# davdwan21/Silent-Speech

Hardware: AMD Instinct MI355X
Metric: clips/sec (30-frame, fwd+bwd) (higher is better)
Workload: dtype f32; 1 GPU; BASELINE config 2: landmark (K=40, D=84) + 64x64 uint8 ROI CNN + 2-layer BiGRU(192), T=30, C=5, train step = fwd + CE(ls .05) + bwd + grad all-reduce + clip(1.0) + Adam, dropout on; batch_per_gpu=256, global_batch=256, frames=30, parallelism=dp1, micro_batches_in_flight=1

## Files before the change

### include/ss_hotpath.h

```cpp
#ifndef SS_HOTPATH_H
#define SS_HOTPATH_H

#include <stdint.h>

#ifdef __cplusplus
extern "C" {
#endif

typedef void* ss_stream_t;

enum ss_status {
  SS_OK = 0,
  SS_ERR_ARG = -1,
  SS_ERR_LAUNCH = -2,
  SS_ERR_UNSUPPORTED = -3
};

int ss_abi_version(void);
const char* ss_status_string(int status);

int ss_feature_fuse(const float* lm, const uint8_t* reset, int B, int T, int K, int w, int h, int a_left,
                    int a_right, int a_up, int a_lo, int variant, float* X, int ldx, float* center,
                    double* fourth, ss_stream_t stream);

// ... 220 lines not shown
                const float* beta, const float* w1, const float* b1, const float* w4, const float* b4, const int64_t* y,
                int B, int T, int D, int MID, int C, float ln_eps, float drop_p, uint64_t seed, uint64_t offset,
                float label_smoothing, float denom, float* attn, float* xhat, float* rstd, float* ln, float* mid,
                float* mid_d, float* logits, float* d_logits, float* loss_sum, int32_t* correct, ss_stream_t stream);
int ss_tail_fwd_w(const float* h, const int32_t* lengths, const float* w_score, const float* b_score, const float* gamma,
                  const float* beta, const float* w1, const float* b1, const float* w4, const float* b4, const int64_t* y,
                  int B, int T, int D, int MID, int C, float ln_eps, float drop_p, uint64_t seed, uint64_t offset,
                  float label_smoothing, const float* cw, const float* den, float* attn, float* xhat, float* rstd, float* ln,
                  float* mid, float* mid_d, float* logits, float* d_logits, float* loss_sum, int32_t* correct,
                  ss_stream_t stream);
int ss_tail_bwd(const float* h, const int32_t* lengths, const float* w_score, const float* gamma, const float* w1,
                const float* w4, const float* attn, const float* xhat, const float* rstd, const float* mid,
                const float* d_logits, int B, int T, int D, int MID, int C, float drop_p, uint64_t seed,
                uint64_t offset, float* d_mid, float* d_h, float* g_gamma, float* g_beta, float* g_wscore,
                float* g_bscore, float* col_part, ss_stream_t stream);

int ss_ce_ls_fwd_bwd(const float* logits, const int64_t* y, int B, int C, float label_smoothing, float denom,
                     float* d_logits, float* loss_sum, int32_t* correct, ss_stream_t stream);

int ss_ce_ls_w_fwd_bwd(const float* logits, const int64_t* y, int B, int C, float label_smoothing, const float* w,
                       const float* den, float* d_logits, float* loss_sum, int32_t* correct, ss_stream_t stream);
int ss_class_weight_sum(const int64_t* y, long n, const float* w, int C, float* out, ss_stream_t stream);

int ss_eval_accum(const float* logits, const int64_t* y, int B, int C, float label_smoothing, int first_row,
                  float* loss_sum, int32_t* correct, int32_t* confusion, int32_t* first_seen, int32_t* y_true_out,
                  int32_t* y_pred_out, int32_t* err_flag, ss_stream_t stream);

int ss_eval_accum_w(const float* logits, const int64_t* y, int B, int C, float label_smoothing, int first_row, const float* w,
                    float* loss_sum, float* wsum, int32_t* correct, int32_t* confusion, int32_t* first_seen,
                    int32_t* y_true_out, int32_t* y_pred_out, int32_t* err_flag, ss_stream_t stream);
// ... 15 lines not shown
```

### silent_speech_amd/_lib.py

```python
from __future__ import annotations

import ctypes as C
import os

import torch

_HERE = os.path.dirname(os.path.abspath(__file__))
LIB_PATH = os.environ.get("SS_HOTPATH_LIB", os.path.join(_HERE, "libss_hotpath.so"))

_vp = C.c_void_p
_i = C.c_int
_f = C.c_float
_l = C.c_long
_u64 = C.c_uint64
_d = C.c_double

SIGNATURES = {
    "ss_abi_version": [],
    "ss_status_string": [_i],
    "ss_feature_fuse": [_vp, _vp, _i, _i, _i, _i, _i, _i, _i, _i, _i, _i, _vp, _i, _vp, _vp, _vp],
    "ss_feature_fuse_stream": [_vp, _vp, _vp, _i, _i, _i, _i, _i, _i, _i, _i, _i, _i, _d, _d, _vp, _vp, _vp, _i, _vp, _vp, _vp, _vp],
    "ss_roi_norm": [_vp, _i, _i, _i, _vp, _vp, _vp],
    "ss_im2col3x3": [_vp, _i, _i, _i, _i, _vp, _i, _vp],
    "ss_relu_pool2": [_vp, _i, _i, _i, _i, _vp, _vp, _vp],
# ... 62 lines not shown
    "ss_ring_push": [_vp, _vp, _i, _i, _i, _i, _vp, _i, _vp, _vp, _vp, _vp, _vp, _vp],
    "ss_ring_window_map": [_vp, _i, _i, _vp, _vp, _vp, _vp, _vp],
    "ss_mouth_openness": [_vp, _i, _i, _i, _i, _i, _i, _i, _vp, _vp],
    "ss_mouth_gate": [_vp, _i, _vp, _d, _d, _d, _vp, _vp, _vp],
    "ss_clip_gate": [_vp, _i, _vp, _vp, _d, _i, _i, _i, _i, _vp, _i, _i, _vp, _vp, _vp, _vp, _vp, _vp, _vp],
    "ss_gru_fwd": [_vp, _vp, _vp, _vp, _vp, _vp, _i, _i, _i, _vp, _vp, _vp, _vp],
    "ss_gru_fwd_drop": [_vp, _vp, _vp, _vp, _vp, _vp, _i, _i, _i, _vp, _vp, _vp, _f, _u64, _u64, _vp, _vp],
    "ss_gru_sync_bytes": [_i, _i, _i, _vp],
    "ss_gru_bwd": [_vp, _vp, _vp, _vp, _vp, _vp, _i, _i, _i, _vp, _f, _u64, _u64, _vp, _vp, _vp, _vp, _vp, _vp],
    "ss_gru_bias_grad": [_vp, _i, _i, _vp, _vp, _vp, _vp, _vp],
    "ss_attn_pool_fwd": [_vp, _vp, _vp, _vp, _i, _i, _i, _vp, _vp, _vp],
    "ss_attn_pool_bwd": [_vp, _vp, _vp, _vp, _vp, _i, _i, _i, _vp, _vp, _vp, _vp],
    "ss_tail_fwd": [_vp] * 11 + [_i] * 5 + [_f, _f, _u64, _u64, _f, _f] + [_vp] * 10 + [_vp],
    "ss_tail_fwd_w": [_vp] * 11 + [_i] * 5 + [_f, _f, _u64, _u64, _f, _vp, _vp] + [_vp] * 10 + [_vp],
    "ss_tail_bwd": [_vp] * 11 + [_i] * 5 + [_f, _u64, _u64] + [_vp] * 7 + [_vp],
    "ss_layernorm_fwd": [_vp, _vp, _vp, _i, _i, _f, _vp, _vp, _vp, _vp],
    "ss_layernorm_bwd": [_vp, _vp, _vp, _vp, _i, _i, _vp, _vp, _vp, _vp],
    "ss_dropout": [_vp, _vp, _l, _f, _u64, _u64, _vp, _vp],
    "ss_ce_ls_fwd_bwd": [_vp, _vp, _i, _i, _f, _f, _vp, _vp, _vp, _vp],
    "ss_eval_accum": [_vp, _vp, _i, _i, _f, _i, _vp, _vp, _vp, _vp, _vp, _vp, _vp, _vp],
    "ss_ce_ls_w_fwd_bwd": [_vp, _vp, _i, _i, _f, _vp, _vp, _vp, _vp, _vp, _vp],
    "ss_class_weight_sum": [_vp, _l, _vp, _i, _vp, _vp],
    "ss_eval_accum_w": [_vp, _vp, _i, _i, _f, _i, _vp, _vp, _vp, _vp, _vp, _vp, _vp, _vp, _vp, _vp],
    "ss_softmax_topk": [_vp, _i, _i, _i, _vp, _vp, _vp],
    "ss_sumsq_f32": [_vp, _l, _vp, _vp],
    "ss_adam_clip": [_vp, _vp, _vp, _vp, _l, _vp, _f, _f, _f, _f, _f, _f, _i, _vp],
    "ss_copy_rows_f32": [_vp, _i, _vp, _i, _i, _i, _vp],
}
_RESTYPES = {"ss_status_string": C.c_char_p}

# ... 110 lines not shown
```

### silent_speech_amd/csrc/tail.hip

```cpp
#include "ss_common.h"
#include "ce_row.h"

namespace {

constexpr int TNT = 1024;
constexpr int NWT = TNT / 64;


__device__ __forceinline__ float drop_scale(long idx, float p, uint64_t seed, uint64_t offset) {
  if (p <= 0.f) return 1.f;
  uint32_t rnd[4];
  const uint64_t ctr = offset + (uint64_t)(idx >> 2);
  philox4((uint32_t)ctr, (uint32_t)(ctr >> 32), 0u, 0u, (uint32_t)seed, (uint32_t)(seed >> 32), rnd);
  const uint32_t thr = (uint32_t)((double)p * 4294967296.0);
  return rnd[idx & 3] >= thr ? 1.0f / (1.0f - p) : 0.f;
}

__device__ __forceinline__ float block_sum(float v, float* red) {
  v = wave_sum(v);
  __syncthreads();
  if ((threadIdx.x & 63) == 0) red[threadIdx.x >> 6] = v;
  __syncthreads();
  float s = 0.f;
#pragma unroll
// ... 7 lines not shown
  const float *w_score, *b_score, *gamma, *beta, *w1, *b1, *w4, *b4;
  const int64_t* y;
  int B, T, D, MID, C;
  float eps, drop_p, ls, denom;
  uint64_t seed, offset;
  float *attn, *xhat, *rstd, *ln, *mid, *mid_d, *logits, *d_logits, *loss_sum;
  int* correct;
  static constexpr bool weighted = false;
};

struct TailFwdParamsW : TailFwdParams {
  const float *cw, *den;
  static constexpr bool weighted = true;
};

template <class Params>
__global__ __launch_bounds__(TNT) void tail_fwd_kernel(Params p) {
  extern __shared__ __attribute__((aligned(16))) float sm[];
  __shared__ float red[2 * NWT];
  const int T = p.T, D = p.D, MID = p.MID, C = p.C;
  float* sc = sm;
  float* pooled = sc + T;
  float* lnv = pooled + D;
  float* midv = lnv + D;
  float* lg = midv + MID;
  const int b = blockIdx.x, tid = threadIdx.x, lane = tid & 63, wv = tid >> 6;
  const int len = p.lengths[b];
  const float* hb = p.h + (long)b * T * D;

  constexpr int PF_PASS = 2, PF_IT = 6, PF_CH = 4;
  float wreg[PF_PASS][4][PF_IT];
#pragma unroll
  for (int ps = 0; ps < PF_PASS; ++ps)
#pragma unroll
// ... 3 lines not shown
        const int o = 4 * wv + u + 4 * NWT * ps, d = lane + 64 * it;
        wreg[ps][u][it] = (o < MID && d < D) ? p.w1[(long)o * D + d] : 0.f;
      }

  const float bsc = p.b_score[0];
  for (int t = wv; t < T; t += NWT) {
    float s = -1e9f;
    if (t < len) {
      s = 0.f;
      float hv[PF_IT], sw[PF_IT];
#pragma unroll
      for (int it = 0; it < PF_IT; ++it) {
        const int d = lane + 64 * it;
        hv[it] = d < D ? hb[(long)t * D + d] : 0.f;
        sw[it] = d < D ? p.w_score[d] : 0.f;
      }
#pragma unroll
      for (int it = 0; it < PF_IT; ++it) s += hv[it] * sw[it];
      for (int d0 = lane + 64 * PF_IT; d0 < D; d0 += 64 * PF_CH) {
        float h2[PF_CH], w2[PF_CH];
#pragma unroll
        for (int it = 0; it < PF_CH; ++it) {
          const int d = d0 + 64 * it;
          h2[it] = d < D ? hb[(long)t * D + d] : 0.f;
          w2[it] = d < D ? p.w_score[d] : 0.f;
        }
#pragma unroll
        for (int it = 0; it < PF_CH; ++it) s += h2[it] * w2[it];
      }
      s = wave_sum(s) + bsc;
    }
    if (lane == 0) sc[t] = s;
  }
  __syncthreads();
  float m = -3.4e38f;
  for (int t = tid; t < T; t += TNT) m = fmaxf(m, sc[t]);
  m = wave_max(m);
  if (lane == 0) red[wv] = m;
  __syncthreads();
  m = red[0];
// ... 4 lines not shown
    const float e = expf(sc[t] - m);
    sc[t] = e;
    sum += e;
  }
  sum = block_sum(sum, red + NWT);
  const float inv = 1.0f / sum;
  for (int t = tid; t < T; t += TNT) {
    const float wt = sc[t] * inv;
    sc[t] = wt;
    if (p.attn) p.attn[(long)b * T + t] = wt;
  }
  __syncthreads();
  float s1 = 0.f;
  for (int d = tid; d < D; d += TNT) {
    float acc = 0.f;
    for (int t = 0; t < len; ++t) acc += sc[t] * hb[(long)t * D + d];
    pooled[d] = acc;
    s1 += acc;
  }
  const float mean = block_sum(s1, red) / D;
  float s2 = 0.f;
  for (int d = tid; d < D; d += TNT) {
    const float c = pooled[d] - mean;
    s2 += c * c;
  }
  const float rs = rsqrtf(block_sum(s2, red + NWT) / D + p.eps);
  for (int d = tid; d < D; d += TNT) {
    const float xh = (pooled[d] - mean) * rs;
    const float v = xh * p.gamma[d] + p.beta[d];
    lnv[d] = v;
    if (p.xhat) p.xhat[(long)b * D + d] = xh;
    if (p.ln) p.ln[(long)b * D + d] = v;
  }
  if (p.rstd && tid == 0) p.rstd[b] = rs;
  __syncthreads();
  float xv[PF_IT];
#pragma unroll
  for (int it = 0; it < PF_IT; ++it) xv[it] = (lane + 64 * it < D) ? lnv[lane + 64 * it] : 0.f;
  int ps = 0;
  for (int o0 = 4 * wv; o0 < MID; o0 += 4 * NWT, ++ps) {
    float acc[4] = {0.f, 0.f, 0.f, 0.f};
    if (ps < PF_PASS) {
#pragma unroll
      for (int it = 0; it < PF_IT; ++it)
#pragma unroll
        for (int u = 0; u < 4; ++u) acc[u] += (ps == 0 ? wreg[0][u][it] : wreg[1][u][it]) * xv[it];
    }
    for (int d0 = lane + (ps < PF_PASS ? 64 * PF_IT : 0); d0 < D; d0 += 64 * PF_CH) {
      float w2[PF_CH][4];
// ... 5 lines not shown
          w2[it][u] = (d < D && o0 + u < MID) ? p.w1[(long)(o0 + u) * D + d] : 0.f;
        }
#pragma unroll
      for (int it = 0; it < PF_CH; ++it) {
        const int d = d0 + 64 * it;
        const float x = d < D ? lnv[d] : 0.f;
#pragma unroll
        for (int u = 0; u < 4; ++u) acc[u] += w2[it][u] * x;
      }
    }
#pragma unroll
    for (int u = 0; u < 4; ++u) acc[u] = wave_sum(acc[u]);
    if (lane < 4 && o0 + lane < MID) {
      const int o = o0 + lane;
      const float a = relu_f((lane == 0 ? acc[0] : lane == 1 ? acc[1] : lane == 2 ? acc[2] : acc[3]) + p.b1[o]);
      const float ad = a * drop_scale((long)b * MID + o, p.drop_p, p.seed, p.offset);
      midv[o] = ad;
      if (p.mid) p.mid[(long)b * MID + o] = a;
      if (p.mid_d) p.mid_d[(long)b * MID + o] = ad;
    }
  }
  __syncthreads();
  for (int c = wv; c < C; c += NWT) {
    float acc = 0.f;
    const float* wr = p.w4 + (long)c * MID;
    for (int o = lane; o < MID; o += 64) acc += wr[o] * midv[o];
    acc = wave_sum(acc);
    if (lane == 0) {
      const float v = acc + p.b4[c];
      lg[c] = v;
      p.logits[(long)b * C + c] = v;
    }
  }
  if (!p.y) return;
  __syncthreads();
  if (wv == 0) {
    float* d_row = p.d_logits + (long)b * C;
    float denom = p.denom;
    const float* cw = nullptr;
    bool valid = true;
    if constexpr (Params::weighted) {
      denom = p.den[0];
      cw = p.cw;
      valid = p.y[b] >= 0 && p.y[b] < (int64_t)C;
    }
    if (valid) {
      const int yy = (int)p.y[b];
      int am;
      const float loss = ce_row_wave<Params::weighted>(lg, yy, C, lane, p.ls, cw, denom, d_row, &am);
      if (lane == 0) {
        if (p.loss_sum) atomicAdd(p.loss_sum, loss / denom);
        if (p.correct && am == yy) atomicAdd(p.correct, 1);
      }
    } else {
      for (int c = lane; c < C; c += 64) d_row[c] = 0.f;
    }
  }
}

struct TailBwdParams {
  const float* h;
  const int* lengths;
  const float *w_score, *gamma, *w1, *w4;
  const float *attn, *xhat, *rstd, *mid, *d_logits;
  int B, T, D, MID, C;
  float drop_p;
  uint64_t seed, offset;
  float *d_mid, *d_h, *g_gamma, *g_beta, *g_wscore, *g_bscore;
  float* col_part;
};

__global__ __launch_bounds__(TNT) void tail_bwd_kernel(TailBwdParams p) {
  extern __shared__ __attribute__((aligned(16))) float sm[];
  __shared__ float red[2 * NWT];
  const int T = p.T, D = p.D, MID = p.MID, C = p.C;
  float* dmid = sm;
  float* dp = dmid + MID;
  float* ds = dp + D;
  float* wt = ds + T;
  float* dl = wt + T;
  const int b = blockIdx.x, tid = threadIdx.x, lane = tid & 63, wv = tid >> 6;
  const int len = p.lengths[b];
  const float* hb = p.h + (long)b * T * D;

  for (int c = tid; c < C; c += TNT) dl[c] = p.d_logits[(long)b * C + c];
  for (int t = tid; t < T; t += TNT) wt[t] = p.attn[(long)b * T + t];
  __syncthreads();
  for (int o = tid; o < MID; o += TNT) {
    float acc = 0.f;
#pragma unroll 16
    for (int c = 0; c < C; ++c) acc += dl[c] * p.w4[(long)c * MID + o];
    acc *= drop_scale((long)b * MID + o, p.drop_p, p.seed, p.offset);
    if (p.mid[(long)b * MID + o] <= 0.f) acc = 0.f;
    dmid[o] = acc;
    p.d_mid[(long)b * MID + o] = acc;
  }
  __syncthreads();
  float s1 = 0.f, s2 = 0.f;
  for (int d = tid; d < D; d += TNT) {
    float acc = 0.f;
#pragma unroll 16
    for (int o = 0; o < MID; ++o) acc += dmid[o] * p.w1[(long)o * D + d];
    const float xh = p.xhat[(long)b * D + d];
    if (p.col_part) {
      p.col_part[((long)b * 3 + 0) * D + d] = acc * xh;
      p.col_part[((long)b * 3 + 1) * D + d] = acc;
    } else {
      atomicAdd(&p.g_gamma[d], acc * xh);
      atomicAdd(&p.g_beta[d], acc);
    }
    const float dxh = acc * p.gamma[d];
    dp[d] = dxh;
    s1 += dxh;
    s2 += dxh * xh;
  }
  s1 = block_sum(s1, red) / D;
  s2 = block_sum(s2, red + NWT) / D;
  const float rs = p.rstd[b];
  for (int d = tid; d < D; d += TNT) dp[d] = rs * (dp[d] - s1 - p.xhat[(long)b * D + d] * s2);
  __syncthreads();
  for (int t = wv; t < T; t += NWT) {
    float c = 0.f;
    if (t < len) {
      for (int d = lane; d < D; d += 64) c += hb[(long)t * D + d] * dp[d];
      c = wave_sum(c);
    }
    if (lane == 0) ds[t] = c;
  }
  __syncthreads();
  float part = 0.f;
  for (int t = tid; t < len; t += TNT) part += wt[t] * ds[t];
  const float dot = block_sum(part, red);
  for (int t = tid; t < T; t += TNT) ds[t] = (t < len) ? wt[t] * (ds[t] - dot) : 0.f;
  __syncthreads();
  for (int d = tid; d < D; d += TNT) {
    const float dpd = dp[d], wd = p.w_score[d];
    float gw = 0.f;
#pragma unroll 8
    for (int t = 0; t < len; ++t) gw += ds[t] * hb[(long)t * D + d];
    for (int t = 0; t < T; ++t) p.d_h[((long)b * T + t) * D + d] = (t < len) ? wt[t] * dpd + ds[t] * wd : 0.f;
    if (p.col_part) p.col_part[((long)b * 3 + 2) * D + d] = gw;
    else atomicAdd(&p.g_wscore[d], gw);
  }
  if (tid == 0) {
    float gb = 0.f;
    for (int t = 0; t < len; ++t) gb += ds[t];
    atomicAdd(p.g_bscore, gb);
  }
}

}

static int tail_fwd_launch(const float* h, const int32_t* lengths, const float* w_score, const float* b_score,
                           const float* gamma, const float* beta, const float* w1, const float* b1, const float* w4,
                           const float* b4, const int64_t* y, int B, int T, int D, int MID, int C, float ln_eps,
                           float drop_p, uint64_t seed, uint64_t offset, float label_smoothing, float denom,
                           const float* cw, const float* den, float* attn, float* xhat, float* rstd, float* ln, float* mid,
                           float* mid_d, float* logits, float* d_logits, float* loss_sum, int32_t* correct,
                           ss_stream_t stream) {
  SS_REQUIRE(h && lengths && w_score && b_score && gamma && beta && w1 && b1 && w4 && b4 && logits, SS_ERR_ARG);
  SS_REQUIRE(B > 0 && T > 0 && D > 0 && MID > 0 && C > 0 && drop_p >= 0.f && drop_p < 1.f, SS_ERR_ARG);
  SS_REQUIRE(!y || (d_logits && denom > 0.f), SS_ERR_ARG);
  const size_t lds = (size_t)(T + 2 * D + MID + C) * sizeof(float);
// ... 44 lines not shown
                           float* g_wscore, float* g_bscore, float* col_part, ss_stream_t stream) {
  SS_REQUIRE(h && lengths && w_score && gamma && w1 && w4 && attn && xhat && rstd && mid && d_logits, SS_ERR_ARG);
  SS_REQUIRE(d_mid && d_h && g_gamma && g_beta && g_wscore && g_bscore, SS_ERR_ARG);
  SS_REQUIRE(B > 0 && T > 0 && D > 0 && MID > 0 && C > 0 && drop_p >= 0.f && drop_p < 1.f, SS_ERR_ARG);
  const size_t lds = (size_t)(MID + D + 2 * T + C) * sizeof(float);
  SS_REQUIRE(lds <= 60 * 1024, SS_ERR_UNSUPPORTED);
  TailBwdParams p;
  p.h = h; p.lengths = lengths; p.w_score = w_score; p.gamma = gamma; p.w1 = w1; p.w4 = w4;
  p.attn = attn; p.xhat = xhat; p.rstd = rstd; p.mid = mid; p.d_logits = d_logits;
  p.B = B; p.T = T; p.D = D; p.MID = MID; p.C = C; p.drop_p = drop_p; p.seed = seed; p.offset = offset;
  p.d_mid = d_mid; p.d_h = d_h; p.g_gamma = g_gamma; p.g_beta = g_beta; p.g_wscore = g_wscore; p.g_bscore = g_bscore;
  p.col_part = col_part;
  hipLaunchKernelGGL(tail_bwd_kernel, dim3(B), dim3(TNT), lds, static_cast<hipStream_t>(stream), p);
  return ss_launch_status();
}
```

### silent_speech_amd/engine.py

```python
from __future__ import annotations

import os

from dataclasses import dataclass
from typing import Dict, Optional

import torch

from . import _lib as L

INT_MAX = 2**31 - 1
_HH_TARGET = 512
USE_SIDE_STREAM = True


@dataclass
class Config:
    x_dim: int
    num_classes: int
    use_roi: bool
    roi_emb: int = 32
    hidden: int = 192
    gru_layers: int = 2
    roi_standardize: bool = True
# ... 117 lines not shown
class Workspace:

    bf16 = False

    def __init__(self, cfg: Config, B: int, T: int, roi_hw, device, train: bool, slot=0):
        self.cfg, self.B, self.T, self.roi_hw, self.train = cfg, B, T, roi_hw, train
        self.stash_gen, self.stash_live = 0, False
        N, H = B * T, cfg.hidden
        f32 = dict(device=device, dtype=torch.float32)
        u8 = dict(device=device, dtype=torch.uint8)
        self.lengths = torch.empty(B, device=device, dtype=torch.int32)
        nb = L.gru_sync_bytes(B, T, H)
        self.gru_sync = torch.zeros(nb // 4, device=device, dtype=torch.int32) if nb else None
        self.side = side_stream(device, slot) if train else None
        self.ev_fork = torch.cuda.Event() if train else None
        self.ev_join = torch.cuda.Event() if train else None
        self.ev_cnn_fwd = torch.cuda.Event() if train else None
        self.stagger = False
        self.Z = torch.empty(N, cfg.in_dim, **f32) if cfg.use_roi and roi_hw is not None else None
        self.cnn_generic = None
        if cfg.use_roi and roi_hw is not None:
            from . import cnn_generic

            if not cnn_generic.fused_supported(*roi_hw):
                self.cnn_generic = cnn_generic.GenericCnn(N, roi_hw[0], roi_hw[1], device, train)
        self.gi = [torch.empty(2, N, 3 * H, **f32) for _ in range(cfg.gru_layers)]
        self.out = [torch.empty(N, 2 * H, **f32) for _ in range(cfg.gru_layers)]
        self.attn = torch.empty(B, T, **f32)
        self.pooled = torch.empty(B, 2 * H, **f32)
        self.ln = torch.empty(B, 2 * H, **f32)
# ... 27 lines not shown
                n_a1, n_a2, n_i1, n_i2, n_m3, n_feat = self.cnn_sizes
                self.st_a1 = torch.empty(N, n_a1, **f32)
                self.st_i1 = torch.empty(N, n_i1, **u8)
                self.st_a2 = torch.empty(N, n_a2, **f32)
                self.st_i2 = torch.empty(N, n_i2, **u8)
                self.st_m3 = torch.empty(N, n_m3, **u8)
                self.st_feat = torch.empty(N, n_feat, **f32)
        self.frames = (torch.empty(1 + N, device=device, dtype=torch.int32)
                       if cfg.use_roi and roi_hw is not None and self.cnn_generic is None and SKIP_PADDED_FRAMES else None)
        self.frames_seen = (torch.full((1,), -1, dtype=torch.int32).pin_memory()
                            if self.frames is not None and train else None)
        self.walk_listed = self.frames is not None


def forward(P: Dict[str, torch.Tensor], cfg: Config, ws: Workspace, X: torch.Tensor, R: Optional[torch.Tensor], *,
            train: bool, stash: bool = False, seed: int = 0, ce=None, x_in_place: bool = False, z_ready: bool = False) -> torch.Tensor:
    if ws.bf16:
        from . import engine_bf16

        return engine_bf16.forward(P, cfg, ws, X, R, train=train, stash=stash, seed=seed, ce=ce, x_in_place=x_in_place)
    B, T, H, N = ws.B, ws.T, cfg.hidden, ws.B * ws.T
    s = L.stream()
    if stash and not ws.train:
        raise RuntimeError("stash=True needs a training workspace")
    if z_ready:
        if stash or train or not cfg.use_roi or X.shape[2] != cfg.in_dim:
            raise RuntimeError("z_ready: inference on rows of width in_dim = x_dim + roi_emb of a use_roi model")
        layer_in, ld_in = X.data_ptr(), cfg.in_dim
    elif cfg.use_roi:
        Hh, Ww = ws.roi_hw
        ws_Z = ws.Z
# ... 30 lines not shown
        fused_drop = drop and ws.gru_sync is not None
        L.call("ss_gru_fwd_drop", ws.gi[l].data_ptr(), P[f"gru.weight_hh_l{l}"].data_ptr(),
               P[f"gru.weight_hh_l{l}_reverse"].data_ptr(), P[f"gru.bias_hh_l{l}"].data_ptr(),
               P[f"gru.bias_hh_l{l}_reverse"].data_ptr(), ws.lengths.data_ptr(), B, T, H, ws.out[l].data_ptr(),
               ws.save[l].data_ptr() if stash else None, ws.out_drop[l].data_ptr() if fused_drop else None,
               cfg.gru_dropout if fused_drop else 0.0, seed, (l + 1) << 40, L.ptr(ws.gru_sync), s, tag="ss_gru_fwd")
        layer_in, ld_in = ws.out[l].data_ptr(), 2 * H
        if drop:
            if not fused_drop:
                L.call("ss_dropout", ws.out[l].data_ptr(), ws.out_drop[l].data_ptr(), N * 2 * H, cfg.gru_dropout, seed,
                       (l + 1) << 40, None, s)
            layer_in = ws.out_drop[l].data_ptr()
    top = ws.out[cfg.gru_layers - 1]
    p_drop = cfg.head_dropout if train else 0.0
    y_ptr, ls, denom, loss_ptr, correct_ptr, cw_ptr, den_ptr = (tuple(ce) + (None, None))[:7] if ce is not None else (None, 0.0, 1.0, None, None, None, None)
    tail_fwd, ce_norm = ("ss_tail_fwd_w", (cw_ptr, den_ptr)) if cw_ptr else ("ss_tail_fwd", (denom,))
    L.call(tail_fwd, top.data_ptr(), ws.lengths.data_ptr(), P["pool.score.weight"].data_ptr(),
           P["pool.score.bias"].data_ptr(), P["head.0.weight"].data_ptr(), P["head.0.bias"].data_ptr(),
           P["head.1.weight"].data_ptr(), P["head.1.bias"].data_ptr(), P["head.4.weight"].data_ptr(),
           P["head.4.bias"].data_ptr(), y_ptr, B, T, 2 * H, cfg.head_mid, cfg.num_classes, cfg.ln_eps, p_drop, seed,
           7 << 40, ls, *ce_norm, ws.attn.data_ptr() if stash else None, ws.xhat.data_ptr() if stash else None,
           ws.rstd.data_ptr() if stash else None, ws.ln.data_ptr() if stash else None,
           ws.mid.data_ptr() if stash else None, ws.mid_drop.data_ptr() if stash else None, ws.logits.data_ptr(),
           ws.d_logits.data_ptr() if ce is not None else None, loss_ptr, correct_ptr, s)
    return ws.logits


def backward(P: Dict[str, torch.Tensor], G: Dict[str, torch.Tensor], cfg: Config, ws: Workspace, X: torch.Tensor,
             R: Optional[torch.Tensor], d_logits: torch.Tensor, *, train: bool, seed: int = 0,
             d_X: Optional[torch.Tensor] = None) -> None:
    if ws.bf16:
        from . import engine_bf16

        return engine_bf16.backward(P, G, cfg, ws, X, R, d_logits, train=train, seed=seed, d_X=d_X)
    B, T, H, N = ws.B, ws.T, cfg.hidden, ws.B * ws.T
    s = L.stream()
    C, MID = cfg.num_classes, cfg.head_mid
    p_drop = cfg.head_dropout if train else 0.0
    top = ws.out[cfg.gru_layers - 1]
    L.call("ss_tail_bwd", top.data_ptr(), ws.lengths.data_ptr(), P["pool.score.weight"].data_ptr(),
           P["head.0.weight"].data_ptr(), P["head.1.weight"].data_ptr(), P["head.4.weight"].data_ptr(),
           ws.attn.data_ptr(), ws.xhat.data_ptr(), ws.rstd.data_ptr(), ws.mid.data_ptr(), d_logits.data_ptr(), B, T,
           2 * H, MID, C, p_drop, seed, 7 << 40, ws.d_mid.data_ptr(), ws.d_out.data_ptr(),
           G["head.0.weight"].data_ptr(), G["head.0.bias"].data_ptr(), G["pool.score.weight"].data_ptr(),
           G["pool.score.bias"].data_ptr(), ws.tail_part.data_ptr(), s)
    side = ws.side if USE_SIDE_STREAM else torch.cuda.current_stream()
    ws.ev_fork.record()

    def head_side_work():
        with torch.cuda.stream(side):
            side.wait_event(ws.ev_fork)
            zero_buffers(ws.d_lower[1:] + ([ws.dZ] if cfg.use_roi else []))
            ws.ev_zero.record()
            if ws.frames_seen is not None:
                ws.frames_seen.copy_(ws.frames[:1], non_blocking=True)
            for k_, name_ in enumerate(("head.0.weight", "head.0.bias", "pool.score.weight")):
                L.call("ss_colsum_f32", _addr(ws.tail_part, k_ * 2 * H), B, 2 * H, 3 * 2 * H, G[name_].data_ptr(), L.stream())
            gemm(0, 0, C, MID, B, d_logits.data_ptr(), C, ws.mid_drop.data_ptr(), MID, G["head.4.weight"].data_ptr(), MID,
                 accumulate=True, atomic=True, a_colsum=G["head.4.bias"].data_ptr())
            gemm(0, 0, MID, 2 * H, B, ws.d_mid.data_ptr(), MID, ws.ln.data_ptr(), 2 * H, G["head.1.weight"].data_ptr(),
                 2 * H, accumulate=True, atomic=True, a_colsum=G["head.1.bias"].data_ptr())

    use_drop = train and cfg.gru_dropout > 0.0
    zero_waited = False
    for l in range(cfg.gru_layers - 1, -1, -1):
        K = cfg.in_dim if l == 0 else 2 * H
# ... 70 lines not shown
```

### silent_speech_amd/train.py

```python
from __future__ import annotations

from typing import Optional

import numpy as np
import torch

from . import _lib as L
from . import engine as E
from .model import BiGRUClassifier


def shard_range(n_items: int, rank: int, world: int):
    per = (n_items + world - 1) // world
    lo = min(n_items, rank * per)
    return lo, min(n_items, lo + per)


def allreduce_flat_grads(flat: torch.Tensor, group=None, always: bool = False) -> None:
    import torch.distributed as dist

    if dist.is_available() and dist.is_initialized() and (always or dist.get_world_size(group) > 1):
        dist.all_reduce(flat, op=dist.ReduceOp.SUM, group=group)


# ... 6 lines not shown
        w64 = np.asarray(class_weights, dtype=np.float64)
    except (TypeError, ValueError) as e:
        raise ValueError(f"class_weights must be a sequence of {num_classes} numbers") from e
    if w64.shape != (num_classes,):
        raise ValueError(f"class_weights must hold one weight per class: shape ({num_classes},), not {w64.shape}")
    with np.errstate(over="ignore"):
        w = w64.astype(np.float32)
    if not (np.isfinite(w).all() and (w > 0).all()):
        raise ValueError("class_weights must be finite and strictly positive")
    return np.ascontiguousarray(w)


class Trainer:

    CNN_RESERVED_CUS = 32

    def __init__(self, model: BiGRUClassifier, lr: float = 3e-4, max_norm: float = 1.0,
                 label_smoothing: float = 0.05, betas=(0.9, 0.999), eps: float = 1e-8, world_size: int = 1,
                 process_group=None, dropout: bool = True, micro_batches: int = 1, always_allreduce: bool = False,
                 class_weights=None):
        cw = None if class_weights is None else check_class_weights(class_weights, model.cfg.num_classes)
        if model.flat_params is None or not model.flat_params.is_cuda:
            raise RuntimeError("Trainer needs the model on a HIP device")
        L.load()
        self.model, self.lr, self.max_norm, self.ls = model, lr, max_norm, label_smoothing
        self.betas, self.eps = betas, eps
        self.world, self.group = world_size, process_group
        self.always_allreduce = always_allreduce
        self.allreduce_events = None
        self.dropout = dropout
# ... 105 lines not shown
        n_el = model.flat_grads.numel()
        L.call("ss_sumsq_f32", model.flat_grads.data_ptr(), n_el, self.scal.data_ptr() + 4, s)
        L.call("ss_adam_clip", model.flat_params.data_ptr(), model.flat_grads.data_ptr(), self.m.data_ptr(),
               self.v.data_ptr(), n_el, self.scal.data_ptr() + 4, 1.0, self.max_norm, self.lr, self.betas[0],
               self.betas[1], self.eps, self.step_count, s)
        return self.scal[0], self.correct[0]

    def _fwd_bwd(self, X, lengths, R, y, denom, train, seed, slot, phase, prologue_done=False):
        model, cfg = self.model, self.model.cfg
        ws = model._workspace(X, R, train=True, slot=slot)
        P = model._param_dict()
        if phase in ("fwd", "both"):
            if not prologue_done:
                ws.lengths.copy_(lengths.to(torch.int32), non_blocking=True)
            E.forward(P, cfg, ws, X, R, train=train, stash=True, seed=seed, x_in_place=prologue_done,
                      ce=(y.data_ptr(), self.ls, denom, self.scal.data_ptr(), self.correct.data_ptr()) + self._ce_w)
        if phase in ("bwd", "both"):
            E.backward(P, self.G, cfg, ws, X, R, ws.d_logits, train=train, seed=seed)

    def grad_norm(self) -> torch.Tensor:
        return self.scal[1].sqrt()
```

Measured before the change: 133,900 clips/s.

## Fuse tail forward, loss and tail backward into one kernel

Adds a combined tail training kernel that runs the attention pooling, LayerNorm, MLP head, label-smoothed CE and the tail backward in one block per sample. Intermediates such as xhat, rstd, mid, the dropout keep mask and d_logits stay in LDS instead of going through global memory. When LDS allows, the sample's hidden rows are also cached in LDS so the three later passes over h skip global reads. This removes a kernel launch and the stash writes and reads, and avoids recomputing the Philox dropout mask. In exchange the kernel asks for up to 128KB of dynamic LDS per block, which may lower occupancy. Backward then waits on a new event instead of launching the tail backward itself.

```diff
diff --git a/include/ss_hotpath.h b/include/ss_hotpath.h
--- a/include/ss_hotpath.h
+++ b/include/ss_hotpath.h
@@ -258,6 +258,19 @@
                 const float* d_logits, int B, int T, int D, int MID, int C, float drop_p, uint64_t seed,
                 uint64_t offset, float* d_mid, float* d_h, float* g_gamma, float* g_beta, float* g_wscore,
                 float* g_bscore, float* col_part, ss_stream_t stream);
+int ss_tail_train(const float* h, const int32_t* lengths, const float* w_score, const float* b_score, const float* gamma,
+                  const float* beta, const float* w1, const float* b1, const float* w4, const float* b4, const int64_t* y,
+                  int B, int T, int D, int MID, int C, float ln_eps, float drop_p, uint64_t seed, uint64_t offset,
+                  float label_smoothing, float denom, float* attn, float* xhat, float* rstd, float* ln, float* mid,
+                  float* mid_d, float* logits, float* d_logits, float* loss_sum, int32_t* correct, float* d_mid, float* d_h,
+                  float* g_gamma, float* g_beta, float* g_wscore, float* g_bscore, float* col_part, ss_stream_t stream);
+int ss_tail_train_w(const float* h, const int32_t* lengths, const float* w_score, const float* b_score, const float* gamma,
+                    const float* beta, const float* w1, const float* b1, const float* w4, const float* b4, const int64_t* y,
+                    int B, int T, int D, int MID, int C, float ln_eps, float drop_p, uint64_t seed, uint64_t offset,
+                    float label_smoothing, const float* cw, const float* den, float* attn, float* xhat, float* rstd,
+                    float* ln, float* mid, float* mid_d, float* logits, float* d_logits, float* loss_sum, int32_t* correct,
+                    float* d_mid, float* d_h, float* g_gamma, float* g_beta, float* g_wscore, float* g_bscore,
+                    float* col_part, ss_stream_t stream);
 
 int ss_ce_ls_fwd_bwd(const float* logits, const int64_t* y, int B, int C, float label_smoothing, float denom,
                      float* d_logits, float* loss_sum, int32_t* correct, ss_stream_t stream);
diff --git a/silent_speech_amd/_lib.py b/silent_speech_amd/_lib.py
--- a/silent_speech_amd/_lib.py
+++ b/silent_speech_amd/_lib.py
@@ -100,6 +100,8 @@
     "ss_tail_fwd": [_vp] * 11 + [_i] * 5 + [_f, _f, _u64, _u64, _f, _f] + [_vp] * 10 + [_vp],
     "ss_tail_fwd_w": [_vp] * 11 + [_i] * 5 + [_f, _f, _u64, _u64, _f, _vp, _vp] + [_vp] * 10 + [_vp],
     "ss_tail_bwd": [_vp] * 11 + [_i] * 5 + [_f, _u64, _u64] + [_vp] * 7 + [_vp],
+    "ss_tail_train": [_vp] * 11 + [_i] * 5 + [_f, _f, _u64, _u64, _f, _f] + [_vp] * 10 + [_vp] * 7 + [_vp],
+    "ss_tail_train_w": [_vp] * 11 + [_i] * 5 + [_f, _f, _u64, _u64, _f, _vp, _vp] + [_vp] * 10 + [_vp] * 7 + [_vp],
     "ss_layernorm_fwd": [_vp, _vp, _vp, _i, _i, _f, _vp, _vp, _vp, _vp],
     "ss_layernorm_bwd": [_vp, _vp, _vp, _vp, _i, _i, _vp, _vp, _vp, _vp],
     "ss_dropout": [_vp, _vp, _l, _f, _u64, _u64, _vp, _vp],
diff --git a/silent_speech_amd/csrc/tail.hip b/silent_speech_amd/csrc/tail.hip
--- a/silent_speech_amd/csrc/tail.hip
+++ b/silent_speech_amd/csrc/tail.hip
@@ -45,10 +45,13 @@
   static constexpr bool weighted = true;
 };
 
-template <class Params>
-__global__ __launch_bounds__(TNT) void tail_fwd_kernel(Params p) {
-  extern __shared__ __attribute__((aligned(16))) float sm[];
-  __shared__ float red[2 * NWT];
+struct TailHand {
+  float *xhat, *rstd, *mid, *scale, *dl, *hs;
+};
+
+
+template <class Params, int MODE>
+__device__ __forceinline__ void tail_fwd_body(const Params& p, float* sm, float* red, const TailHand& hd) {
   const int T = p.T, D = p.D, MID = p.MID, C = p.C;
   float* sc = sm;
   float* pooled = sc + T;
@@ -82,6 +85,7 @@
         const int d = lane + 64 * it;
         hv[it] = d < D ? hb[(long)t * D + d] : 0.f;
         sw[it] = d < D ? p.w_score[d] : 0.f;
+        if (MODE == 2 && d < D) hd.hs[t * D + d] = hv[it];
       }
 #pragma unroll
       for (int it = 0; it < PF_IT; ++it) s += hv[it] * sw[it];
@@ -92,6 +96,7 @@
           const int d = d0 + 64 * it;
           h2[it] = d < D ? hb[(long)t * D + d] : 0.f;
           w2[it] = d < D ? p.w_score[d] : 0.f;
+          if (MODE == 2 && d < D) hd.hs[t * D + d] = h2[it];
         }
 #pragma unroll
         for (int it = 0; it < PF_CH; ++it) s += h2[it] * w2[it];
@@ -126,7 +131,11 @@
   float s1 = 0.f;
   for (int d = tid; d < D; d += TNT) {
     float acc = 0.f;
-    for (int t = 0; t < len; ++t) acc += sc[t] * hb[(long)t * D + d];
+    if (MODE == 2) {
+      for (int t = 0; t < len; ++t) acc += sc[t] * hd.hs[t * D + d];
+    } else {
+      for (int t = 0; t < len; ++t) acc += sc[t] * hb[(long)t * D + d];
+    }
     pooled[d] = acc;
     s1 += acc;
   }
@@ -141,10 +150,12 @@
     const float xh = (pooled[d] - mean) * rs;
     const float v = xh * p.gamma[d] + p.beta[d];
     lnv[d] = v;
+    if (MODE > 0) hd.xhat[d] = xh;
     if (p.xhat) p.xhat[(long)b * D + d] = xh;
     if (p.ln) p.ln[(long)b * D + d] = v;
   }
   if (p.rstd && tid == 0) p.rstd[b] = rs;
+  if (MODE > 0 && tid == 0) hd.rstd[0] = rs;
   __syncthreads();
   float xv[PF_IT];
 #pragma unroll
@@ -180,8 +191,13 @@
     if (lane < 4 && o0 + lane < MID) {
       const int o = o0 + lane;
       const float a = relu_f((lane == 0 ? acc[0] : lane == 1 ? acc[1] : lane == 2 ? acc[2] : acc[3]) + p.b1[o]);
-      const float ad = a * drop_scale((long)b * MID + o, p.drop_p, p.seed, p.offset);
+      const float keep = drop_scale((long)b * MID + o, p.drop_p, p.seed, p.offset);
+      const float ad = a * keep;
       midv[o] = ad;
+      if (MODE > 0) {
+        hd.mid[o] = a;
+        hd.scale[o] = keep;
+      }
       if (p.mid) p.mid[(long)b * MID + o] = a;
       if (p.mid_d) p.mid_d[(long)b * MID + o] = ad;
     }
@@ -201,7 +217,8 @@
   if (!p.y) return;
   __syncthreads();
   if (wv == 0) {
-    float* d_row = p.d_logits + (long)b * C;
+    float* d_out_row = p.d_logits + (long)b * C;
+    float* d_row = MODE > 0 ? hd.dl : d_out_row;
     float denom = p.denom;
     const float* cw = nullptr;
     bool valid = true;
@@ -221,7 +238,16 @@
     } else {
       for (int c = lane; c < C; c += 64) d_row[c] = 0.f;
     }
-  }
+    if (MODE > 0)
+      for (int c = lane; c < C; c += 64) d_out_row[c] = d_row[c];
+  }
+}
+
+template <class Params>
+__global__ __launch_bounds__(TNT) void tail_fwd_kernel(Params p) {
+  extern __shared__ __attribute__((aligned(16))) float sm[];
+  __shared__ float red[2 * NWT];
+  tail_fwd_body<Params, 0>(p, sm, red, TailHand{});
 }
 
 struct TailBwdParams {
@@ -236,28 +262,29 @@
   float* col_part;
 };
 
-__global__ __launch_bounds__(TNT) void tail_bwd_kernel(TailBwdParams p) {
-  extern __shared__ __attribute__((aligned(16))) float sm[];
-  __shared__ float red[2 * NWT];
+template <int MODE>
+__device__ __forceinline__ void tail_bwd_body(const TailBwdParams& p, float* sm, float* wt, float* dl, float* red,
+                                              const TailHand& hd) {
   const int T = p.T, D = p.D, MID = p.MID, C = p.C;
   float* dmid = sm;
   float* dp = dmid + MID;
   float* ds = dp + D;
-  float* wt = ds + T;
-  float* dl = wt + T;
   const int b = blockIdx.x, tid = threadIdx.x, lane = tid & 63, wv = tid >> 6;
   const int len = p.lengths[b];
   const float* hb = p.h + (long)b * T * D;
-
-  for (int c = tid; c < C; c += TNT) dl[c] = p.d_logits[(long)b * C + c];
-  for (int t = tid; t < T; t += TNT) wt[t] = p.attn[(long)b * T + t];
+  const float* xrow = MODE > 0 ? hd.xhat : p.xhat + (long)b * D;
+
+  if (MODE == 0) {
+    for (int c = tid; c < C; c += TNT) dl[c] = p.d_logits[(long)b * C + c];
+    for (int t = tid; t < T; t += TNT) wt[t] = p.attn[(long)b * T + t];
+  }
   __syncthreads();
   for (int o = tid; o < MID; o += TNT) {
     float acc = 0.f;
 #pragma unroll 16
     for (int c = 0; c < C; ++c) acc += dl[c] * p.w4[(long)c * MID + o];
-    acc *= drop_scale((long)b * MID + o, p.drop_p, p.seed, p.offset);
-    if (p.mid[(long)b * MID + o] <= 0.f) acc = 0.f;
+    acc *= MODE > 0 ? hd.scale[o] : drop_scale((long)b * MID + o, p.drop_p, p.seed, p.offset);
+    if ((MODE > 0 ? hd.mid[o] : p.mid[(long)b * MID + o]) <= 0.f) acc = 0.f;
     dmid[o] = acc;
     p.d_mid[(long)b * MID + o] = acc;
   }
@@ -267,7 +294,7 @@
     float acc = 0.f;
 #pragma unroll 16
     for (int o = 0; o < MID; ++o) acc += dmid[o] * p.w1[(long)o * D + d];
-    const float xh = p.xhat[(long)b * D + d];
+    const float xh = xrow[d];
     if (p.col_part) {
       p.col_part[((long)b * 3 + 0) * D + d] = acc * xh;
       p.col_part[((long)b * 3 + 1) * D + d] = acc;
@@ -282,13 +309,17 @@
   }
   s1 = block_sum(s1, red) / D;
   s2 = block_sum(s2, red + NWT) / D;
-  const float rs = p.rstd[b];
-  for (int d = tid; d < D; d += TNT) dp[d] = rs * (dp[d] - s1 - p.xhat[(long)b * D + d] * s2);
+  const float rs = MODE > 0 ? hd.rstd[0] : p.rstd[b];
+  for (int d = tid; d < D; d += TNT) dp[d] = rs * (dp[d] - s1 - xrow[d] * s2);
   __syncthreads();
   for (int t = wv; t < T; t += NWT) {
     float c = 0.f;
     if (t < len) {
-      for (int d = lane; d < D; d += 64) c += hb[(long)t * D + d] * dp[d];
+      if (MODE == 2) {
+        for (int d = lane; d < D; d += 64) c += hd.hs[t * D + d] * dp[d];
+      } else {
+        for (int d = lane; d < D; d += 64) c += hb[(long)t * D + d] * dp[d];
+      }
       c = wave_sum(c);
     }
     if (lane == 0) ds[t] = c;
@@ -302,8 +333,13 @@
   for (int d = tid; d < D; d += TNT) {
     const float dpd = dp[d], wd = p.w_score[d];
     float gw = 0.f;
+    if (MODE == 2) {
 #pragma unroll 8
-    for (int t = 0; t < len; ++t) gw += ds[t] * hb[(long)t * D + d];
+      for (int t = 0; t < len; ++t) gw += ds[t] * hd.hs[t * D + d];
+    } else {
+#pragma unroll 8
+      for (int t = 0; t < len; ++t) gw += ds[t] * hb[(long)t * D + d];
+    }
     for (int t = 0; t < T; ++t) p.d_h[((long)b * T + t) * D + d] = (t < len) ? wt[t] * dpd + ds[t] * wd : 0.f;
     if (p.col_part) p.col_part[((long)b * 3 + 2) * D + d] = gw;
     else atomicAdd(&p.g_wscore[d], gw);
@@ -313,6 +349,42 @@
     for (int t = 0; t < len; ++t) gb += ds[t];
     atomicAdd(p.g_bscore, gb);
   }
+}
+
+__global__ __launch_bounds__(TNT) void tail_bwd_kernel(TailBwdParams p) {
+  extern __shared__ __attribute__((aligned(16))) float sm[];
+  __shared__ float red[2 * NWT];
+  float* wt = sm + p.MID + p.D + p.T;
+  tail_bwd_body<0>(p, sm, wt, wt + p.T, red, TailHand{});
+}
+
+struct TailTrainParams {
+  TailFwdParamsW f;
+  TailBwdParams g;
+};
+
+constexpr size_t tail_train_lds_floats(int T, int D, int MID, int C) {
+  return (size_t)(T + 2 * D + MID + C) + D + 2 * MID + C + 4 + (MID + D + T);
+}
+
+template <bool WEIGHTED, bool KEEP>
+__global__ __launch_bounds__(TNT) void tail_train_kernel(TailTrainParams p) {
+  extern __shared__ __attribute__((aligned(16))) float sm[];
+  __shared__ float red[2 * NWT];
+  const int T = p.f.T, D = p.f.D, MID = p.f.MID, C = p.f.C;
+  constexpr int MODE = KEEP ? 2 : 1;
+  float* fwd = sm;
+  TailHand hd;
+  hd.xhat = fwd + T + 2 * D + MID + C;
+  hd.mid = hd.xhat + D;
+  hd.scale = hd.mid + MID;
+  hd.dl = hd.scale + MID;
+  hd.rstd = hd.dl + C;
+  float* bwd = hd.rstd + 4;
+  hd.hs = bwd + MID + D + T;
+  if constexpr (WEIGHTED) tail_fwd_body<TailFwdParamsW, MODE>(p.f, fwd, red, hd);
+  else tail_fwd_body<TailFwdParams, MODE>(static_cast<const TailFwdParams&>(p.f), fwd, red, hd);
+  tail_bwd_body<MODE>(p.g, bwd, fwd , hd.dl, red, hd);
 }
 
 }
@@ -387,3 +459,72 @@
   hipLaunchKernelGGL(tail_bwd_kernel, dim3(B), dim3(TNT), lds, static_cast<hipStream_t>(stream), p);
   return ss_launch_status();
 }
+
+constexpr int TAIL_TRAIN_LDS = 128 * 1024;
+
+template <bool WEIGHTED, bool KEEP>
+static int tail_train_go(const TailTrainParams& p, size_t lds, hipStream_t stream) {
+  const int st = ss_dynamic_lds(reinterpret_cast<const void*>(&tail_train_kernel<WEIGHTED, KEEP>), TAIL_TRAIN_LDS);
+  if (st != SS_OK) return st;
+  hipLaunchKernelGGL((tail_train_kernel<WEIGHTED, KEEP>), dim3(p.f.B), dim3(TNT), lds, stream, p);
+  return ss_launch_status();
+}
+
+static int tail_train_launch(const float* h, const int32_t* lengths, const float* w_score, const float* b_score,
+                             const float* gamma, const float* beta, const float* w1, const float* b1, const float* w4,
+                             const float* b4, const int64_t* y, int B, int T, int D, int MID, int C, float ln_eps,
+                             float drop_p, uint64_t seed, uint64_t offset, float label_smoothing, float denom,
+                             const float* cw, const float* den, float* attn, float* xhat, float* rstd, float* ln, float* mid,
+                             float* mid_d, float* logits, float* d_logits, float* loss_sum, int32_t* correct, float* d_mid,
+                             float* d_h, float* g_gamma, float* g_beta, float* g_wscore, float* g_bscore, float* col_part,
+                             ss_stream_t stream) {
+  SS_REQUIRE(h && lengths && w_score && b_score && gamma && beta && w1 && b1 && w4 && b4 && y && logits && d_logits, SS_ERR_ARG);
+  SS_REQUIRE(d_mid && d_h && g_gamma && g_beta && g_wscore && g_bscore, SS_ERR_ARG);
+  SS_REQUIRE(B > 0 && T > 0 && D > 0 && MID > 0 && C > 0 && drop_p >= 0.f && drop_p < 1.f && denom > 0.f, SS_ERR_ARG);
+  const size_t base = tail_train_lds_floats(T, D, MID, C) * sizeof(float), rows = (size_t)T * D * sizeof(float);
+  SS_REQUIRE(base <= (size_t)TAIL_TRAIN_LDS, SS_ERR_UNSUPPORTED);
+  const bool keep = base + rows <= (size_t)TAIL_TRAIN_LDS;
+  const size_t lds = keep ? base + rows : base;
+  TailTrainParams p;
+  p.f.cw = cw; p.f.den = den;
+  p.f.h = h; p.f.lengths = lengths; p.f.w_score = w_score; p.f.b_score = b_score; p.f.gamma = gamma; p.f.beta = beta;
+  p.f.w1 = w1; p.f.b1 = b1; p.f.w4 = w4; p.f.b4 = b4; p.f.y = y;
+  p.f.B = B; p.f.T = T; p.f.D = D; p.f.MID = MID; p.f.C = C;
+  p.f.eps = ln_eps; p.f.drop_p = drop_p; p.f.ls = label_smoothing; p.f.denom = denom; p.f.seed = seed; p.f.offset = offset;
+  p.f.attn = attn; p.f.xhat = xhat; p.f.rstd = rstd; p.f.ln = ln; p.f.mid = mid; p.f.mid_d = mid_d; p.f.logits = logits;
+  p.f.d_logits = d_logits; p.f.loss_sum = loss_sum; p.f.correct = correct;
+  p.g.h = h; p.g.lengths = lengths; p.g.w_score = w_score; p.g.gamma = gamma; p.g.w1 = w1; p.g.w4 = w4;
+  p.g.attn = nullptr; p.g.xhat = nullptr; p.g.rstd = nullptr; p.g.mid = nullptr; p.g.d_logits = nullptr;
+  p.g.B = B; p.g.T = T; p.g.D = D; p.g.MID = MID; p.g.C = C; p.g.drop_p = drop_p; p.g.seed = seed; p.g.offset = offset;
+  p.g.d_mid = d_mid; p.g.d_h = d_h; p.g.g_gamma = g_gamma; p.g.g_beta = g_beta; p.g.g_wscore = g_wscore;
+  p.g.g_bscore = g_bscore; p.g.col_part = col_part;
+  hipStream_t s = static_cast<hipStream_t>(stream);
+  if (cw) return keep ? tail_train_go<true, true>(p, lds, s) : tail_train_go<true, false>(p, lds, s);
+  return keep ? tail_train_go<false, true>(p, lds, s) : tail_train_go<false, false>(p, lds, s);
+}
+
+extern "C" int ss_tail_train(const float* h, const int32_t* lengths, const float* w_score, const float* b_score,
+                             const float* gamma, const float* beta, const float* w1, const float* b1, const float* w4,
+                             const float* b4, const int64_t* y, int B, int T, int D, int MID, int C, float ln_eps,
+                             float drop_p, uint64_t seed, uint64_t offset, float label_smoothing, float denom,
+                             float* attn, float* xhat, float* rstd, float* ln, float* mid, float* mid_d, float* logits,
+                             float* d_logits, float* loss_sum, int32_t* correct, float* d_mid, float* d_h, float* g_gamma,
+                             float* g_beta, float* g_wscore, float* g_bscore, float* col_part, ss_stream_t stream) {
+  return tail_train_launch(h, lengths, w_score, b_score, gamma, beta, w1, b1, w4, b4, y, B, T, D, MID, C, ln_eps, drop_p, seed,
+                           offset, label_smoothing, denom, nullptr, nullptr, attn, xhat, rstd, ln, mid, mid_d, logits, d_logits,
+                           loss_sum, correct, d_mid, d_h, g_gamma, g_beta, g_wscore, g_bscore, col_part, stream);
+}
+
+extern "C" int ss_tail_train_w(const float* h, const int32_t* lengths, const float* w_score, const float* b_score,
+                               const float* gamma, const float* beta, const float* w1, const float* b1, const float* w4,
+                               const float* b4, const int64_t* y, int B, int T, int D, int MID, int C, float ln_eps,
+                               float drop_p, uint64_t seed, uint64_t offset, float label_smoothing, const float* cw,
+                               const float* den, float* attn, float* xhat, float* rstd, float* ln, float* mid, float* mid_d,
+                               float* logits, float* d_logits, float* loss_sum, int32_t* correct, float* d_mid, float* d_h,
+                               float* g_gamma, float* g_beta, float* g_wscore, float* g_bscore, float* col_part,
+                               ss_stream_t stream) {
+  SS_REQUIRE(cw && den, SS_ERR_ARG);
+  return tail_train_launch(h, lengths, w_score, b_score, gamma, beta, w1, b1, w4, b4, y, B, T, D, MID, C, ln_eps, drop_p, seed,
+                           offset, label_smoothing, 1.0f, cw, den, attn, xhat, rstd, ln, mid, mid_d, logits, d_logits, loss_sum,
+                           correct, d_mid, d_h, g_gamma, g_beta, g_wscore, g_bscore, col_part, stream);
+}
diff --git a/silent_speech_amd/engine.py b/silent_speech_amd/engine.py
--- a/silent_speech_amd/engine.py
+++ b/silent_speech_amd/engine.py
@@ -155,6 +155,8 @@
         self.gru_sync = torch.zeros(nb // 4, device=device, dtype=torch.int32) if nb else None
         self.side = side_stream(device, slot) if train else None
         self.ev_fork = torch.cuda.Event() if train else None
+        self.ev_tail = torch.cuda.Event() if train else None
+        self.tail_done = False
         self.ev_join = torch.cuda.Event() if train else None
         self.ev_cnn_fwd = torch.cuda.Event() if train else None
         self.stagger = False
@@ -212,7 +214,8 @@
 
 
 def forward(P: Dict[str, torch.Tensor], cfg: Config, ws: Workspace, X: torch.Tensor, R: Optional[torch.Tensor], *,
-            train: bool, stash: bool = False, seed: int = 0, ce=None, x_in_place: bool = False, z_ready: bool = False) -> torch.Tensor:
+            train: bool, stash: bool = False, seed: int = 0, ce=None, x_in_place: bool = False, z_ready: bool = False,
+            grads: Optional[Dict[str, torch.Tensor]] = None) -> torch.Tensor:
     if ws.bf16:
         from . import engine_bf16
 
@@ -273,12 +276,27 @@
     top = ws.out[cfg.gru_layers - 1]
     p_drop = cfg.head_dropout if train else 0.0
     y_ptr, ls, denom, loss_ptr, correct_ptr, cw_ptr, den_ptr = (tuple(ce) + (None, None))[:7] if ce is not None else (None, 0.0, 1.0, None, None, None, None)
+    fused = grads is not None
+    if fused and (ce is None or not stash):
+        raise RuntimeError("grads= needs ce= and stash=True: the fused tail runs the loss and its backward")
     tail_fwd, ce_norm = ("ss_tail_fwd_w", (cw_ptr, den_ptr)) if cw_ptr else ("ss_tail_fwd", (denom,))
-    L.call(tail_fwd, top.data_ptr(), ws.lengths.data_ptr(), P["pool.score.weight"].data_ptr(),
-           P["pool.score.bias"].data_ptr(), P["head.0.weight"].data_ptr(), P["head.0.bias"].data_ptr(),
-           P["head.1.weight"].data_ptr(), P["head.1.bias"].data_ptr(), P["head.4.weight"].data_ptr(),
-           P["head.4.bias"].data_ptr(), y_ptr, B, T, 2 * H, cfg.head_mid, cfg.num_classes, cfg.ln_eps, p_drop, seed,
-           7 << 40, ls, *ce_norm, ws.attn.data_ptr() if stash else None, ws.xhat.data_ptr() if stash else None,
+    fwd_args = (top.data_ptr(), ws.lengths.data_ptr(), P["pool.score.weight"].data_ptr(),
+                P["pool.score.bias"].data_ptr(), P["head.0.weight"].data_ptr(), P["head.0.bias"].data_ptr(),
+                P["head.1.weight"].data_ptr(), P["head.1.bias"].data_ptr(), P["head.4.weight"].data_ptr(),
+                P["head.4.bias"].data_ptr(), y_ptr, B, T, 2 * H, cfg.head_mid, cfg.num_classes, cfg.ln_eps, p_drop, seed,
+                7 << 40, ls, *ce_norm)
+    ws.tail_done = False
+    if fused:
+        G = grads
+        L.call("ss_tail_train_w" if cw_ptr else "ss_tail_train", *fwd_args, None, None, None, ws.ln.data_ptr(), None,
+               ws.mid_drop.data_ptr(), ws.logits.data_ptr(), ws.d_logits.data_ptr(), loss_ptr, correct_ptr,
+               ws.d_mid.data_ptr(), ws.d_out.data_ptr(), G["head.0.weight"].data_ptr(), G["head.0.bias"].data_ptr(),
+               G["pool.score.weight"].data_ptr(), G["pool.score.bias"].data_ptr(), ws.tail_part.data_ptr(), s,
+               tag="ss_tail_train")
+        ws.ev_tail.record()
+        ws.tail_done = True
+        return ws.logits
+    L.call(tail_fwd, *fwd_args, ws.attn.data_ptr() if stash else None, ws.xhat.data_ptr() if stash else None,
            ws.rstd.data_ptr() if stash else None, ws.ln.data_ptr() if stash else None,
            ws.mid.data_ptr() if stash else None, ws.mid_drop.data_ptr() if stash else None, ws.logits.data_ptr(),
            ws.d_logits.data_ptr() if ce is not None else None, loss_ptr, correct_ptr, s)
@@ -297,18 +315,22 @@
     C, MID = cfg.num_classes, cfg.head_mid
     p_drop = cfg.head_dropout if train else 0.0
     top = ws.out[cfg.gru_layers - 1]
-    L.call("ss_tail_bwd", top.data_ptr(), ws.lengths.data_ptr(), P["pool.score.weight"].data_ptr(),
-           P["head.0.weight"].data_ptr(), P["head.1.weight"].data_ptr(), P["head.4.weight"].data_ptr(),
-           ws.attn.data_ptr(), ws.xhat.data_ptr(), ws.rstd.data_ptr(), ws.mid.data_ptr(), d_logits.data_ptr(), B, T,
-           2 * H, MID, C, p_drop, seed, 7 << 40, ws.d_mid.data_ptr(), ws.d_out.data_ptr(),
-           G["head.0.weight"].data_ptr(), G["head.0.bias"].data_ptr(), G["pool.score.weight"].data_ptr(),
-           G["pool.score.bias"].data_ptr(), ws.tail_part.data_ptr(), s)
+    tail_done, ws.tail_done = ws.tail_done, False
+    if not tail_done:
+        L.call("ss_tail_bwd", top.data_ptr(), ws.lengths.data_ptr(), P["pool.score.weight"].data_ptr(),
+               P["head.0.weight"].data_ptr(), P["head.1.weight"].data_ptr(), P["head.4.weight"].data_ptr(),
+               ws.attn.data_ptr(), ws.xhat.data_ptr(), ws.rstd.data_ptr(), ws.mid.data_ptr(), d_logits.data_ptr(), B, T,
+               2 * H, MID, C, p_drop, seed, 7 << 40, ws.d_mid.data_ptr(), ws.d_out.data_ptr(),
+               G["head.0.weight"].data_ptr(), G["head.0.bias"].data_ptr(), G["pool.score.weight"].data_ptr(),
+               G["pool.score.bias"].data_ptr(), ws.tail_part.data_ptr(), s)
     side = ws.side if USE_SIDE_STREAM else torch.cuda.current_stream()
-    ws.ev_fork.record()
+    ev_head = ws.ev_tail if tail_done else ws.ev_fork
+    if not tail_done:
+        ws.ev_fork.record()
 
     def head_side_work():
         with torch.cuda.stream(side):
-            side.wait_event(ws.ev_fork)
+            side.wait_event(ev_head)
             zero_buffers(ws.d_lower[1:] + ([ws.dZ] if cfg.use_roi else []))
             ws.ev_zero.record()
             if ws.frames_seen is not None:
diff --git a/silent_speech_amd/train.py b/silent_speech_amd/train.py
--- a/silent_speech_amd/train.py
+++ b/silent_speech_amd/train.py
@@ -44,6 +44,7 @@
 class Trainer:
 
     CNN_RESERVED_CUS = 32
+    fuse_tail = True
 
     def __init__(self, model: BiGRUClassifier, lr: float = 3e-4, max_norm: float = 1.0,
                  label_smoothing: float = 0.05, betas=(0.9, 0.999), eps: float = 1e-8, world_size: int = 1,
@@ -179,7 +180,8 @@
             if not prologue_done:
                 ws.lengths.copy_(lengths.to(torch.int32), non_blocking=True)
             E.forward(P, cfg, ws, X, R, train=train, stash=True, seed=seed, x_in_place=prologue_done,
-                      ce=(y.data_ptr(), self.ls, denom, self.scal.data_ptr(), self.correct.data_ptr()) + self._ce_w)
+                      ce=(y.data_ptr(), self.ls, denom, self.scal.data_ptr(), self.correct.data_ptr()) + self._ce_w,
+                      grads=self.G if self.fuse_tail else None)
         if phase in ("bwd", "both"):
             E.backward(P, self.G, cfg, ws, X, R, ws.d_logits, train=train, seed=seed)
 
```

Result: no change. 134,300 clips/s (median of 6 runs) (+0.3%).
